# VisualComputingInstitute/diffusion-e2e-ft

Measured on AMD Instinct MI355X. Metric: images/sec (768x768, 1-step UNet fwd) full path: VAE encode + SD-v2 UNet @t=999 + VAE decode, higher is better.
Workload: dtype f16

## Files before the change

### diffusion-e2e-ft_amd/_lib.py

```python
import ctypes as C
import os

import torch

from . import build as _build

_LIB = None

F32, F16, BF16 = 0, 1, 2
_DT = {torch.float32: F32, torch.float16: F16, torch.bfloat16: BF16}


def dtype_id(dt):
    try:
        return _DT[dt]
    except KeyError:
        raise TypeError("libe2eft supports float32/float16/bfloat16, got %s" % dt)


class ConvDesc(C.Structure):
    _fields_ = [(n, C.c_int32) for n in (
        "dtype", "batch", "hin", "win", "hl", "wl", "c1", "ldx1", "c2", "ldx2", "kh", "kw", "stride", "pad_t", "pad_l",
        "hout", "wout", "cout", "ldo", "ldr", "ldw")] + [("alpha", C.c_float)]

# ... 29 lines not shown
class HypersimDesc(C.Structure):
    _fields_ = [(n, C.c_int32) for n in ("batch", "height", "width", "color_dtype", "distance_dtype", "depth_format")] + [
        ("focal", C.c_double), ("scale_numerator", C.c_double)]


HYPERSIM_DEPTH_U16, HYPERSIM_DEPTH_F32 = range(2)
HYPERSIM_RECORD = 16


class DepthGtDesc(C.Structure):
    _fields_ = ([(n, C.c_int32) for n in ("batch", "h0", "w0", "raw_dtype")] + [("divisor", C.c_double)]
                + [(n, C.c_int32) for n in ("inf_to_zero", "crop_top", "crop_left", "crop_h", "crop_w")] + [("min_depth", C.c_float), ("max_depth", C.c_float)]
                + [(n, C.c_int32) for n in ("win_y0", "win_y1", "win_x0", "win_x1", "use_ext_mask")])


GT_U16, GT_I32, GT_F32 = range(3)


class NormalGtDesc(C.Structure):
    _fields_ = [(n, C.c_int32) for n in ("batch", "height", "width", "raw_dtype")]


NORMAL_GT_U8, NORMAL_GT_F32 = range(2)


class DsineRgbDesc(C.Structure):
    _fields_ = [(n, C.c_int32) for n in ("batch", "height", "width", "out_layout")]


RGB_HWC, RGB_CHW = range(2)
DSINE_RGB_WS_INTS = 6


OPT_PERSISTENT, OPT_PERSISTENT_GRID, OPT_NARROW_CONV, OPT_NARROW_MFMA, OPT_IGEMM_GENERAL_OPERANDS, OPT_IGEMM2_WAVES, OPT_PATCH_CONV, OPT_THIN_INPUT_CONV, OPT_FUSED_NORM, OPT_ATTN_DMA, OPT_UPCONV_PHASES, OPT_PATCH_CONV_2X2, OPT_PERSISTENT_MIN_QROUNDS, OPT_GN_APPLY_ITERS, OPT_F32_SPLIT, OPT_F32_SPLIT_ATTN = range(16)

_P = C.c_void_p
_I = C.c_int32
_L = C.c_int64
_F = C.c_float
_Z = C.c_size_t

SIGNATURES = {
    "e2eft_version": (_I, []),
    "e2eft_last_error": (C.c_char_p, []),
    "e2eft_build_id": (C.c_char_p, []),
    "e2eft_set_option": (_I, [_I, _I]),
    "e2eft_get_option": (_I, [_I]),
    "e2eft_conv2d_fwd": (_I, [C.POINTER(ConvDesc), _P, _P, _P, _P, _P, _P, _P, _P]),
    "e2eft_gemm": (_I, [C.POINTER(GemmDesc), _P, _P, _P, _P, _P, _P]),
    "e2eft_conv2d_fwd_gnstats": (_I, [C.POINTER(ConvDesc), _P, _P, _P, _P, _P, _P, _P, _P, _Z, C.POINTER(C.c_int32), _P]),
    "e2eft_conv2d_splitk_workspace_bytes": (_Z, [C.POINTER(ConvDesc)]),
    "e2eft_conv2d_fwd_splitk": (_I, [C.POINTER(ConvDesc), _P, _P, _P, _P, _P, _P, _P, _P, _Z, _P]),
    "e2eft_gemm_gnstats": (_I, [C.POINTER(GemmDesc), _P, _P, _P, _P, _P, _I, _P, _Z, C.POINTER(C.c_int32), _P]),
    "e2eft_groupnorm_fwd_pre": (_I, [C.POINTER(GroupNormDesc), _P, _P, _P, _P, _P, _P, _I, _P, _I, _P, _Z, _P]),
    "e2eft_groupnorm_coeff_offset": (_Z, [C.POINTER(GroupNormDesc)]),
    "e2eft_groupnorm_fwd_stats": (_I, [C.POINTER(GroupNormDesc), _P, _P, _P, _P, _I, _P, _I, _P, _Z, _P]),
    "e2eft_conv2d_fwd_normed_supported": (_I, [C.POINTER(ConvDesc)]),
    "e2eft_upconv2x_fwd_supported": (_I, [C.POINTER(ConvDesc)]),
    "e2eft_upconv2x_fwd": (_I, [C.POINTER(ConvDesc), _P, _P, _P, _P, _P, _Z, C.POINTER(C.c_int32), _P]),
    "e2eft_groupnorm_fwd_split": (_I, [C.POINTER(GroupNormDesc), _P, _P, _P, _P, _I, _P, _P, _I, _P, _Z, _P]),
    "e2eft_f32_split_weight": (_I, [_P, _L, _I, _P, _P, _P]),
    "e2eft_f32_split2_cat": (_I, [_P, _I, _I, _P, _I, _I, _L, _P, _I, _P, _P]),
    "e2eft_f32_split2": (_I, [_P, _L, _I, _I, _P, _I, _P, _P]),
    "e2eft_f32_split2_cols": (_I, [_P, _I, _I, _P, _I, _I, _L, _P, _I, _P, _P]),
    "e2eft_f32_split_wgrad_finish": (_I, [_P, _P, _P, _L, _I, _I, _P, _P, _P, _P]),
    "e2eft_conv2d_fwd_f32split_supported": (_I, [C.POINTER(ConvDesc)]),
    "e2eft_conv2d_fwd_f32split": (_I, [C.POINTER(ConvDesc), _P, _P, _P, _P, _P, _P, _P, _P, _Z, C.POINTER(C.c_int32), _P]),
    "e2eft_upconv2x_fwd_f32split_supported": (_I, [C.POINTER(ConvDesc)]),
    "e2eft_upconv2x_fwd_f32split": (_I, [C.POINTER(ConvDesc), _P, _P, _P, _P, _P, _P, _P, _Z, C.POINTER(C.c_int32), _P]),
    "e2eft_gemm_f32split_supported": (_I, [C.POINTER(GemmDesc)]),
    "e2eft_attn_f32split_supported": (_I, [C.POINTER(AttnDesc), _I]),
    "e2eft_gemm_f32split": (_I, [C.POINTER(GemmDesc), _P, _P, _P, _P, _P, _P, _P, _P]),
    "e2eft_conv2d_fwd_normed": (_I, [C.POINTER(ConvDesc), _P, _P, _P, _I, _P, _P, _P, _P, _P, _P, _Z, C.POINTER(C.c_int32), _P]),
    "e2eft_groupnorm_workspace_bytes": (_Z, [C.POINTER(GroupNormDesc)]),
    "e2eft_groupnorm_fwd": (_I, [C.POINTER(GroupNormDesc), _P, _P, _P, _P, _P, _P, _Z, _P]),
    "e2eft_layernorm_fwd": (_I, [_I, _L, _I, _I, _I, _F, _P, _P, _P, _P, _P]),
    "e2eft_geglu_fwd": (_I, [_I, _L, _I, _I, _I, _P, _P, _P]),
    "e2eft_softmax_rows": (_I, [_I, _L, _I, _L, _F, _P, _P]),
    "e2eft_softmax_rows_causal": (_I, [_I, _L, _I, _L, _F, _I, _P, _P]),
    "e2eft_attn_fwd": (_I, [C.POINTER(AttnDesc), _P, _P, _P, _P, _P]),
    "e2eft_attn_fwd_lse": (_I, [C.POINTER(AttnDesc), _P, _P, _P, _P, _P, _P]),
    "e2eft_attn512_workspace_bytes": (_Z, [C.POINTER(AttnDesc)]),
    "e2eft_attn512_fwd": (_I, [C.POINTER(AttnDesc), _P, _P, _P, _P, _P, _Z, _P]),
    "e2eft_attn_bwd_workspace_bytes": (_Z, [C.POINTER(AttnDesc)]),
    "e2eft_attn_bwd": (_I, [C.POINTER(AttnDesc), _P, _P, _P, _P, _P, _I, _P, _P, _I, _P, _I, _P, _I, _P, _Z, _P]),
    "e2eft_nchw_to_nhwc": (_I, [_I, _I, _I, _I, _I, _I, _I, _F, _F, _P, _P, _P]),
    "e2eft_nhwc_to_nchw": (_I, [_I, _I, _I, _I, _I, _I, _F, _F, _P, _P, _P]),
    "e2eft_copy_scale": (_I, [_I, _L, _I, _I, _I, _F, _F, _P, _P, _P]),
    "e2eft_add": (_I, [_I, _L, _I, _I, _I, _I, _P, _P, _P, _P]),
    "e2eft_timestep_embedding": (_I, [_I, _I, _I, _P, _P, _P]),
    "e2eft_silu": (_I, [_I, _L, _P, _P, _P]),
    "e2eft_depth_head": (_I, [_I, _I, _L, _I, _I, _P, _P, _P]),
    "e2eft_normal_head": (_I, [_I, _I, _I, _I, _I, _I, _F, _P, _P, _P]),
    "e2eft_ssi_loss_workspace_bytes": (_Z, [_I]),
    "e2eft_ssi_loss_fwd": (_I, [_I, _I, _P, _P, _P, _P, _P, _P, _Z, _P]),
    "e2eft_angular_loss_workspace_bytes": (_Z, [_I]),
    "e2eft_angular_loss_fwd": (_I, [_I, _I, _P, _P, _P, _P, _P, _Z, _P]),
    "e2eft_conv2d_dgrad": (_I, [C.POINTER(ConvDesc), _P, _I, _I, _P, _I, _P, _I, _P]),
    "e2eft_conv2d_wgrad_workspace_bytes": (_Z, [C.POINTER(ConvDesc), _I]),
    "e2eft_conv2d_wgrad": (_I, [C.POINTER(ConvDesc), _P, _I, _P, _P, _P, _Z, C.POINTER(C.c_int32), _P]),
    "e2eft_conv2d_im2col_t": (_I, [C.POINTER(ConvDesc), _P, _P, _P, _L, _P]),
    "e2eft_transpose": (_I, [_I, _I, _L, _I, _L, _L, _L, _L, _L, _P, _P, _P]),
    "e2eft_colsum_workspace_bytes": (_Z, [_I, _L, _I]),
    "e2eft_colsum": (_I, [_I, _I, _L, _I, _L, _F, _P, _P, _P, _Z, _P]),
    "e2eft_upsample_nearest_bwd": (_I, [_I, _I, _I, _I, _I, _I, _I, _I, _I, _P, _P, _P]),
    "e2eft_groupnorm_bwd_workspace_bytes": (_Z, [C.POINTER(GroupNormDesc)]),
    "e2eft_groupnorm_bwd": (_I, [C.POINTER(GroupNormDesc), _P, _P, _P, _P, _P, _I, _P, _I, _P, _P, _P, _P, _Z, _P]),
    "e2eft_groupnorm_bwd_add": (_I, [C.POINTER(GroupNormDesc), _P, _P, _P, _P, _P, _I, _P, _I, _P, _I, _P, _P, _P, _P, _Z, _P]),
    "e2eft_layernorm_bwd_workspace_bytes": (_Z, [_L, _I]),
# ... 117 lines not shown
```

### diffusion-e2e-ft_amd/build.py

```python
import hashlib
import os
import shutil
import subprocess
import sys
from concurrent.futures import ThreadPoolExecutor

HERE = os.path.dirname(os.path.abspath(__file__))
CSRC = os.path.join(HERE, "csrc")
LIBDIR = os.path.join(HERE, "lib")
OBJDIR = os.path.join(HERE, "build")
LIB = os.path.join(LIBDIR, "libe2eft.so")
SOURCES = ["api.hip", "igemm.hip", "igemm2.hip", "igemm5.hip", "igemm6.hip", "convin.hip", "norm.hip", "attn.hip", "attn32.hip", "attn512.hip", "attn_bwd.hip", "elementwise.hip", "loss.hip", "bwd.hip", "wgrad.hip", "ensemble.hip", "dataprep.hip", "narrow.hip", "dataaug.hip", "evalmetrics.hip", "normaleval.hip", "d2nt.hip", "hypersimprep.hip", "evalprep.hip", "normalprep.hip", "prepost.hip", "f32split.hip", "attn_f32split.hip", "noise.hip"]
FLAGS = ["--offload-arch=gfx950", "-O3", "-std=c++17", "-fPIC", "-fvisibility=hidden", "-Wall", "-Wno-unused-function"]
EXTRA_FLAGS = {"attn.hip": ["-fno-slp-vectorize"], "attn32.hip": ["-fno-slp-vectorize"], "attn_f32split.hip": ["-fno-slp-vectorize"], "attn512.hip": ["-fno-slp-vectorize"], "igemm.hip": ["-fno-slp-vectorize"], "igemm2.hip": ["-fno-slp-vectorize"], "igemm5.hip": ["-fno-slp-vectorize"], "igemm6.hip": ["-fno-slp-vectorize"], "f32split.hip": ["-fno-slp-vectorize"], "convin.hip": ["-fno-slp-vectorize"],
               "d2nt.hip": ["-ffp-contract=off"],
               "hypersimprep.hip": ["-ffp-contract=off"],
               "evalprep.hip": ["-ffp-contract=off"],
               "normalprep.hip": ["-ffp-contract=off"]}


def _hipcc():
    for cand in (os.environ.get("HIPCC"), shutil.which("hipcc"), "/opt/rocm/bin/hipcc"):
        if cand and os.path.exists(cand):
            return cand
    raise RuntimeError("hipcc not found (need ROCm >= 7.0 to build libe2eft.so for gfx950)")


HEADERS = ["common.h", "gfx950.h", "igemm.h", "attn32.h", "attn512_regs.inc", "igemm_persistent_epilogue.inc"]


def _inputs():
    inc = os.path.join(HERE, "..", "include")
    return [os.path.join(CSRC, f) for f in sorted(SOURCES + HEADERS)] + [os.path.join(inc, "e2eft.h"), os.path.join(inc, "e2eft_debug.h")]


def _newest_source_mtime():
    return max(os.path.getmtime(p) for p in _inputs() + [os.path.abspath(__file__)])


ID_MARK = b"E2EFT_BUILD_ID="


def source_id():
    h = hashlib.sha256()
    for path in _inputs():
# ... 102 lines not shown
```

### diffusion-e2e-ft_amd/csrc/api.hip

```cpp
#include "common.h"
#include <atomic>

namespace e2eft {

static thread_local char g_err[512] = "";

char* err_buf() { return g_err; }

int fail(int code, const char* fmt, ...) {
    va_list ap;
    va_start(ap, fmt);
    vsnprintf(g_err, sizeof(g_err), fmt, ap);
    va_end(ap);
    return code;
}

int check_launch(const char* what) {
    hipError_t e = hipGetLastError();
    if (e != hipSuccess) return fail(E2EFT_ERR_LAUNCH, "%s: launch failed: %s", what, hipGetErrorString(e));
    return E2EFT_OK;
}

static std::atomic<int> g_cus_of_device[64];
int device_cus() {
    int dev = 0;
    if (hipGetDevice(&dev) != hipSuccess || dev < 0 || dev >= 64) return 0;
    int n = g_cus_of_device[dev].load(std::memory_order_relaxed);
    if (n == 0) {
        if (hipDeviceGetAttribute(&n, hipDeviceAttributeMultiprocessorCount, dev) != hipSuccess || n < 8) return 0;
        n &= ~7;
        g_cus_of_device[dev].store(n, std::memory_order_relaxed);
    }
    return n;
}

static thread_local char g_tag[96] = "";
void tag_kernel(const char* fmt, ...) {
    va_list ap;
    va_start(ap, fmt);
    vsnprintf(g_tag, sizeof(g_tag), fmt, ap);
    va_end(ap);
}
const char* last_tag() { return g_tag; }

static std::atomic<int> g_opt[E2EFT_OPT_COUNT] = {{1}, {0}, {1}, {1}, {0}, {0}, {1}, {1}, {1}, {1}, {1}, {1}, {2}, {0}, {1}, {0}};

int option(int key) { return g_opt[key].load(std::memory_order_relaxed); }

}

extern "C" int e2eft_set_option(int32_t key, int32_t value) {
    using namespace e2eft;
    E2EFT_REQUIRE(key >= 0 && key < E2EFT_OPT_COUNT, "set_option: unknown key %d", key);
    bool ok = value == 0 || value == 1;
    if (key == E2EFT_OPT_PERSISTENT_GRID) ok = value == 0 || (value >= 8 && value % 8 == 0 && value <= 4096);
    if (key == E2EFT_OPT_IGEMM2_WAVES) ok = value == 0 || value == 4 || value == 8;
    if (key == E2EFT_OPT_PERSISTENT_MIN_QROUNDS) ok = value >= 1 && value <= 64;
    if (key == E2EFT_OPT_GN_APPLY_ITERS) ok = value >= 0 && value <= 16;
    E2EFT_REQUIRE(ok, "set_option: value %d out of range for key %d", value, key);
    g_opt[key].store(value, std::memory_order_relaxed);
    return E2EFT_OK;
}
extern "C" int e2eft_get_option(int32_t key) { return key >= 0 && key < E2EFT_OPT_COUNT ? e2eft::option(key) : -1; }

extern "C" const char* e2eft_debug_last_kernel(void) { return e2eft::last_tag(); }

extern "C" int e2eft_version(void) { return E2EFT_VERSION; }
#ifndef E2EFT_BUILD_ID
#define E2EFT_BUILD_ID "unstamped"
#endif
static const char k_build_id[] = "E2EFT_BUILD_ID=" E2EFT_BUILD_ID;
extern "C" const char* e2eft_build_id(void) { return k_build_id + 15; }
extern "C" const char* e2eft_last_error(void) { return e2eft::err_buf(); }
```

### diffusion-e2e-ft_amd/modules.py

```python

import torch
from torch import nn

from . import ops
from . import autograd as F


_cached = F.cached


def packed_conv_weight(conv):
    return F.packed_conv_weight(conv, conv.weight.dtype)


def conv_nhwc(conv, x, x2=None, up_to=None, rowadd=None, residual=None, alpha=1.0, pad=None, out=None, gn_stats=True, norm=None):
    assert out is None
    return F.conv(conv, x, x2=x2, up_to=up_to, rowadd=rowadd, residual=residual, alpha=alpha, pad=pad, gn_stats=gn_stats, norm=norm)


def checkpointed(enabled, fn, *args):
    if enabled and torch.is_grad_enabled() and any(isinstance(a, torch.Tensor) and a.requires_grad for a in args):
        from torch.utils.checkpoint import checkpoint
        return checkpoint(fn, *args, use_reentrant=False)
    return fn(*args)
# ... 167 lines not shown
    ops.softmax_rows_(s.view(-1, nkp), nkt, scale)
    o = torch.empty((B, N, C), dtype=dt, device=dev)
    for qh in range(nseg):
        ops.bgemm_raw(dt, N, d, nkp, s[qh * Bv:], nkp, (heads * N * nkp, N * nkp), vt, nkp, (C * nkp, d * nkp), o[qh * Bv:], C, (N * C, d),
                      Bv, heads)
    return o


class Attention(nn.Module):

    def __init__(self, query_dim, heads, cross_attention_dim=None, bias=False, joint=False):
        super().__init__()
        self.heads = heads
        self.scale = (query_dim // heads) ** -0.5
        self.joint = joint
        kv = cross_attention_dim or query_dim
        self.to_q = Linear(query_dim, query_dim, bias=bias)
        self.to_k = Linear(kv, query_dim, bias=bias)
        self.to_v = Linear(kv, query_dim, bias=bias)
        self.to_out = nn.ModuleList([Linear(query_dim, query_dim), nn.Dropout(0.0)])

    def forward(self, x, ctx=None, residual=None):
        B, N, C = x.shape
        d = C // self.heads
        out = self.to_out[0]
        kv_pre = None
        shared_src = None
        if isinstance(ctx, CtxCond):
            kv_pre = ctx.kv.get(id(self))
            shared_src = ctx.src if ctx.shared else None
            ctx = ctx.ctx
        if F.needs_grad(x, ctx, self.to_q.weight, self.to_k.weight, self.to_v.weight, out.weight):
            return out(self._forward_train(x, ctx), residual=residual)
        if (CROSS_ATTN_FOLD and shared_src is not None and shared_src.shape[1] == 2 and not self.joint and self.to_q.bias is None and self.to_k.bias is None
                and self.to_v.bias is None and self.heads <= 64):
            return self._folded(x, shared_src, residual)
        fused = F.fused_attention_ok(x.dtype, d)
        dt = x.dtype
        if fused:
            if ctx is None:
                qkv = F.linear(x, (self.to_q.weight, self.to_k.weight, self.to_v.weight), owner=self, name="wqkv")
                q, k, v = qkv[..., :C], qkv[..., C:2 * C], qkv[..., 2 * C:]
            else:
                q = self.to_q(x)
                kv = kv_pre
                if kv is None or torch.is_grad_enabled():
                    kv = F.linear(ctx, (self.to_k.weight, self.to_v.weight), owner=self, name="wkv")
                k, v = kv[..., :C], kv[..., C:]
            a = ops.attention(q, k, v, self.heads, self.scale, kv_nseg=2 if self.joint else 1, kv_bmod=B // 2 if self.joint else B)
        else:
            src = x if ctx is None else ctx
            cw = lambda lin: F._cat_weight(lin, "w", (lin.weight,), dt, lin.weight.shape[1])
            a = attention_unfused(x, src, cw(self.to_q), F._vec(self.to_q.bias, dt), cw(self.to_k), F._vec(self.to_k.bias, dt), cw(self.to_v),
                                  F._vec(self.to_v.bias, dt), self.heads, self.scale, joint=self.joint)
        return out(a, residual=residual)

    def _fold(self, src, dt):
        out = self.to_out[0]
        ws = [w for w in (self.to_q.weight, self.to_k.weight, self.to_v.weight, out.weight, out.bias) if w is not None]
        key = (src.data_ptr(), src._version, tuple(src.shape), str(src.device), dt, F._key(*ws))
        hit = self.__dict__.get("_fold_cache")
        if hit is not None and hit[0] == key:
            return hit[1]
        with torch.no_grad():
            h, C = self.heads, self.to_q.weight.shape[0]
            d = C // h
            f32 = lambda w: w.detach().float().contiguous()
            wq, wk, wv, wo = f32(self.to_q.weight), f32(self.to_k.weight), f32(self.to_v.weight), f32(out.weight)
            c32 = f32(src[0])
            k = ops.gemm(c32, wk)
            v = ops.gemm(c32, wv)
            ar = torch.arange(h, device=k.device)
            Mk = torch.zeros((h, h, d), dtype=torch.float32, device=k.device)
            Mv = torch.zeros((h, h, d), dtype=torch.float32, device=k.device)
            Mk[ar, ar] = (k[0] - k[1]).view(h, d) * self.scale
            Mv[ar, ar] = (v[0] - v[1]).view(h, d)
            G = ops.gemm(Mk.view(h, C), wq.t().contiguous())
            delta = ops.gemm(Mv.view(h, C), wo)
            c0 = ops.gemm(v[1:2].contiguous(), wo, f32(out.bias) if out.bias is not None else None)[0]
            hp = ops.round_up(h, ops.epc(dt))
            Gp = torch.zeros((hp, C), dtype=torch.float32, device=G.device)
            Gp[:h] = G
            Dt = torch.zeros((C, hp), dtype=torch.float32, device=G.device)
            Dt[:, :h] = delta.t()
            val = (Gp.to(dt).contiguous(), Dt.to(dt).contiguous(), c0.to(dt).contiguous())
        self.__dict__["_fold_cache"] = (key, val, src)
        return val

    def _folded(self, x, src, residual):
        G, Dt, c0 = self._fold(src, x.dtype)
        p = ops.activation(ops.linear(x, G), "sigmoid")
        return ops.linear(p, Dt, c0, residual=residual)

    def _forward_train(self, x, ctx):
        B, N, C = x.shape
        if ctx is None:
            bias = None if self.to_q.bias is None else torch.cat([self.to_q.bias, self.to_k.bias, self.to_v.bias])
            qkv = F.linear(x, (self.to_q.weight, self.to_k.weight, self.to_v.weight), bias, owner=self, name="wqkv")
            if self.joint:
                Bv = B // 2
                q, kv = qkv[..., :C], qkv[..., C:]
                kv = torch.cat([kv[:Bv], kv[Bv:]], dim=1).repeat(2, 1, 1)
                return F.attention(q.contiguous(), kv, self.heads, self.scale)
            return F.attention(qkv, None, self.heads, self.scale)
        q = self.to_q(x)
        bias = None if self.to_k.bias is None else torch.cat([self.to_k.bias, self.to_v.bias])
        kv = F.linear(ctx, (self.to_k.weight, self.to_v.weight), bias, owner=self, name="wkv")
        return F.attention(q, kv, self.heads, self.scale)


class GEGLU(nn.Module):

    def __init__(self, dim, inner):
        super().__init__()
        self.proj = Linear(dim, 2 * inner)

    def forward(self, x):
        return F.geglu(self.proj(x))


class FeedForward(nn.Module):

    def __init__(self, dim):
        super().__init__()
        self.net = nn.ModuleList([GEGLU(dim, 4 * dim), nn.Dropout(0.0), Linear(4 * dim, dim)])

    def forward(self, x, residual=None):
        return self.net[2](self.net[0](x), residual=residual)


class BasicTransformerBlock(nn.Module):

    def __init__(self, dim, heads, cross_attention_dim, joint=False):
        super().__init__()
        self.norm1 = LayerNorm(dim, eps=1e-5)
        self.attn1 = Attention(dim, heads, joint=joint)
        self.norm2 = LayerNorm(dim, eps=1e-5)
        self.attn2 = Attention(dim, heads, cross_attention_dim=cross_attention_dim)
        self.norm3 = LayerNorm(dim, eps=1e-5)
        self.ff = FeedForward(dim)

    def forward(self, h, ctx):
        h = self.attn1(self.norm1(h), None, residual=h)
        h = self.attn2(self.norm2(h), ctx, residual=h)
        return self.ff(self.norm3(h), residual=h)


class Transformer2DModel(nn.Module):

    def __init__(self, channels, heads, cross_attention_dim, groups=32, joint=False):
        super().__init__()
        self.norm = GroupNorm(groups, channels, eps=1e-6, affine=True)
        self.proj_in = Linear(channels, channels)
        self.transformer_blocks = nn.ModuleList([BasicTransformerBlock(channels, heads, cross_attention_dim, joint=joint)])
        self.proj_out = Linear(channels, channels)

    def nhwc(self, x, ctx):
        B, H, W, C = x.shape
        h, x = self.norm.nhwc(x, split=True)
        h = self.proj_in(h.view(B, H * W, C))
        for blk in self.transformer_blocks:
            h = blk(h, ctx)
        out = self.proj_out(h, residual=x.reshape(B, H * W, C), gn_rows_per_image=H * W)
        res = out.view(B, H, W, C)
        st = getattr(out, "_e2eft_gn", None)
        if st is not None:
            res._e2eft_gn = st
        return res


class VaeAttention(nn.Module):

    def __init__(self, channels, groups=32):
        super().__init__()
        self.group_norm = GroupNorm(groups, channels, eps=1e-6, affine=True)
        self.to_q = Linear(channels, channels)
        self.to_k = Linear(channels, channels)
        self.to_v = Linear(channels, channels)
# ... 28 lines not shown
```

### diffusion-e2e-ft_amd/ops.py

```python
import ctypes as C

import torch

from . import _lib
from ._lib import ConvDesc, GemmDesc, GroupNormDesc, AttnDesc, check, dtype_id


class KernelTimer:

    def __init__(self, only=None):
        self.rec = {}
        self.only = only

    def add(self, name, start, end, flops, nbytes, label=None, launches=1, flops_nominal=None):
        self.rec.setdefault(name, []).append((start, end, flops, nbytes, label, launches, flops if flops_nominal is None else flops_nominal))

    def summary(self):
        torch.cuda.synchronize()
        out = {}
        for name, lst in self.rec.items():
            ms = sum(r[0].elapsed_time(r[1]) for r in lst)
            out[name] = dict(launches=sum(r[5] for r in lst), ms=ms, flops=float(sum(r[2] for r in lst)), bytes=float(sum(r[3] for r in lst)),
                             flops_nominal=float(sum(r[6] for r in lst)))
        return out
# ... 579 lines not shown


NORM_FUSION_ENABLED = True


def groupnorm_stats(x, gamma, groups, eps):
    _check_cuda(x, gamma)
    B, H, W, c1 = x.shape
    d = GroupNormDesc()
    d.dtype = dtype_id(x.dtype)
    d.batch, d.hw = B, H * W
    d.c1, d.ldx1, d.c2, d.ldx2 = c1, _nhwc_ld(x), 0, 0
    d.groups, d.ldy, d.silu, d.eps = groups, c1, 0, eps
    lib = _lib.load()
    nbytes = lib.e2eft_groupnorm_workspace_bytes(C.byref(d))
    if nbytes == 0:
        raise RuntimeError("groupnorm_stats: %s" % lib.e2eft_last_error().decode())
    ws = torch.empty((nbytes + 3) // 4, dtype=torch.float32, device=x.device)
    s1 = getattr(x, "_e2eft_gn", None) if GN_STATS_ENABLED else None
    with _timed("groupnorm_stats", 0.0, 0.0, label="gn stats B%d %dx%d C%d" % (B, H, W, c1)):
        check(lib.e2eft_groupnorm_fwd_stats(C.byref(d), _ptr(x), C.c_void_p(0), _ptr(gamma), _ptr(s1.partial) if s1 else C.c_void_p(0), s1.nslabs if s1 else 0,
                                            C.c_void_p(0), 0, _ptr(ws), nbytes, _stream()))
    return ws, ws.data_ptr() + lib.e2eft_groupnorm_coeff_offset(C.byref(d))


def layernorm(x, gamma, beta, eps, out=None):
    _check_cuda(x, gamma, beta, out)
    Cc = x.shape[-1]
    a = x.reshape(-1, Cc) if x.is_contiguous() else _as_rows(x)
    if out is None:
        out = torch.empty(x.shape, dtype=x.dtype, device=x.device)
    o = out.reshape(-1, Cc) if out.is_contiguous() else _as_rows(out)
    assert gamma.dtype == x.dtype and beta.dtype == x.dtype
    check(_lib.load().e2eft_layernorm_fwd(dtype_id(x.dtype), a.shape[0], Cc, _rows_ld(a), _rows_ld(o), eps, _ptr(a), _ptr(gamma),
                                         _ptr(beta), _ptr(o), _stream()))
    return out


def geglu(h, out=None):
    _check_cuda(h, out)
    c2 = h.shape[-1]
    c = c2 // 2
    a = h.reshape(-1, c2) if h.is_contiguous() else _as_rows(h)
    if out is None:
        out = torch.empty((*h.shape[:-1], c), dtype=h.dtype, device=h.device)
    o = out.reshape(-1, c) if out.is_contiguous() else _as_rows(out)
    check(_lib.load().e2eft_geglu_fwd(dtype_id(h.dtype), a.shape[0], c, _rows_ld(a), _rows_ld(o), _ptr(a), _ptr(o), _stream()))
    return out


def softmax_rows_(s, n, scale, causal_nq=0):
    _check_cuda(s)
    assert s.dim() == 2 and s.is_contiguous()
    if causal_nq:
        check(_lib.load().e2eft_softmax_rows_causal(dtype_id(s.dtype), s.shape[0], n, s.shape[1], scale, causal_nq, _ptr(s), _stream()))
    else:
        check(_lib.load().e2eft_softmax_rows(dtype_id(s.dtype), s.shape[0], n, s.shape[1], scale, _ptr(s), _stream()))
    return s


def _ld3(t):
    if t.shape[2] > 1 and t.stride(2) != 1:
        raise ValueError("attention operands need unit inner stride")
    ld = t.stride(1) if t.shape[1] > 1 else max(t.shape[2], t.stride(1))
    if t.shape[0] > 1 and t.stride(0) != t.shape[1] * ld:
        raise ValueError("attention operands must be batch-dense: %s %s" % (tuple(t.shape), t.stride()))
    return ld


def _attn_desc(q, k, v, out, heads, scale, kv_nseg, kv_bmod):
    B, Nq, Wd = q.shape
    Bkv, Nk, _ = k.shape
    assert Wd == heads * 64 and k.shape[2] == Wd and v.shape == k.shape
    d = AttnDesc()
    d.dtype = dtype_id(q.dtype)
    d.batch, d.heads, d.nq, d.nk_seg = B, heads, Nq, Nk
    d.kv_nseg = kv_nseg
    d.kv_bmod = B if kv_bmod is None else kv_bmod
    assert Bkv >= d.kv_bmod * kv_nseg
    d.ldq, d.ldk, d.ldv, d.ldo = _ld3(q), _ld3(k), _ld3(v), _ld3(out)
# ... 118 lines not shown
    _check_cuda(a, b, out)
    assert a.shape == b.shape and a.dtype == b.dtype
    if out is None:
        out = torch.empty(a.shape, dtype=a.dtype, device=a.device)
    Cc = a.shape[-1]
    aa, bb, oo = (_as_rows(t) if t.dim() > 2 else t for t in (a, b, out))
    check(_lib.load().e2eft_add(dtype_id(a.dtype), aa.shape[0], Cc, _rows_ld(aa), _rows_ld(bb), _rows_ld(oo), _ptr(aa), _ptr(bb), _ptr(oo), _stream()))
    return out


def timestep_embedding(t, dim, dtype):
    _check_cuda(t)
    t = t.to(torch.int64).contiguous()
    out = torch.empty((t.shape[0], dim), dtype=dtype, device=t.device)
    check(_lib.load().e2eft_timestep_embedding(dtype_id(dtype), t.shape[0], dim, _ptr(t), _ptr(out), _stream()))
    return out


def silu(x):
    _check_cuda(x)
    x = x.contiguous()
    out = torch.empty_like(x)
    check(_lib.load().e2eft_silu(dtype_id(x.dtype), x.numel(), _ptr(x), _ptr(out), _stream()))
    return out


ACT_KINDS = {"quick_gelu": 0, "gelu": 1, "silu": 2, "sigmoid": 3}


def activation(x, kind):
    _check_cuda(x)
    x = x.contiguous()
    out = torch.empty_like(x)
    check(_lib.load().e2eft_activation(dtype_id(x.dtype), ACT_KINDS[kind], x.numel(), _ptr(x), _ptr(out), _stream()))
    return out


def depth_head(x, to_unit, dtype=None):
    _check_cuda(x)
    B, H, W, _ = x.shape
    dtype = dtype or x.dtype
    y = torch.empty((B, 1, H, W), dtype=dtype, device=x.device)
    mode = 2 if to_unit == "mean" else (1 if to_unit else 0)
    check(_lib.load().e2eft_depth_head(dtype_id(x.dtype), dtype_id(dtype), B * H * W, _nhwc_ld(x), mode, _ptr(x), _ptr(y), _stream()))
    return y


def normal_head(x, clamp=False, sign=1.0, dtype=None):
    _check_cuda(x)
    B, H, W, _ = x.shape
    dtype = dtype or x.dtype
    y = torch.empty((B, 3, H, W), dtype=dtype, device=x.device)
    check(_lib.load().e2eft_normal_head(dtype_id(x.dtype), dtype_id(dtype), B, H * W, _nhwc_ld(x), 1 if clamp else 0, sign, _ptr(x), _ptr(y), _stream()))
    return y


def ssi_loss(pred, target, mask, return_scale_shift=False):
    _check_cuda(pred, target, mask)
    B = pred.shape[0]
    p = pred.reshape(B, -1).float().contiguous()
    t = target.reshape(B, -1).float().contiguous()
    m = mask.reshape(B, -1).to(torch.uint8).contiguous()
    lib = _lib.load()
    nbytes = lib.e2eft_ssi_loss_workspace_bytes(B)
    ws = torch.empty((nbytes + 7) // 8, dtype=torch.float64, device=p.device)
    out = torch.empty(1, dtype=torch.float32, device=p.device)
    ss = torch.empty((B, 2), dtype=torch.float32, device=p.device)
# ... 831 lines not shown
```

### include/e2eft.h

```cpp
#ifndef E2EFT_H
#define E2EFT_H

#include <stddef.h>
#include <stdint.h>

#ifdef __cplusplus
extern "C" {
#endif
#pragma GCC visibility push(default)

#define E2EFT_VERSION 119

enum {
    E2EFT_OK = 0,
    E2EFT_ERR_BAD_ARG = 1,
    E2EFT_ERR_WORKSPACE = 2,
    E2EFT_ERR_LAUNCH = 3,
    E2EFT_ERR_UNSUPPORTED = 4,
};

enum { E2EFT_F32 = 0, E2EFT_F16 = 1, E2EFT_BF16 = 2 };

int e2eft_version(void);
const char* e2eft_last_error(void);
const char* e2eft_build_id(void);

enum {
    E2EFT_OPT_PERSISTENT = 0,
    E2EFT_OPT_PERSISTENT_GRID = 1,
    E2EFT_OPT_NARROW_CONV = 2,
    E2EFT_OPT_NARROW_MFMA = 3,
    E2EFT_OPT_IGEMM_GENERAL_OPERANDS = 4,
    E2EFT_OPT_IGEMM2_WAVES = 5,
    E2EFT_OPT_PATCH_CONV = 6,
    E2EFT_OPT_THIN_INPUT_CONV = 7,
    E2EFT_OPT_FUSED_NORM = 8,
    E2EFT_OPT_ATTN_DMA = 9,
    E2EFT_OPT_UPCONV_PHASES = 10,
    E2EFT_OPT_PATCH_CONV_2X2 = 11,
    E2EFT_OPT_PERSISTENT_MIN_QROUNDS = 12,
    E2EFT_OPT_GN_APPLY_ITERS = 13,
    E2EFT_OPT_F32_SPLIT = 14,
    E2EFT_OPT_F32_SPLIT_ATTN = 15,
    E2EFT_OPT_COUNT = 16
};
int e2eft_set_option(int32_t key, int32_t value);
int e2eft_get_option(int32_t key);

typedef struct E2eftConvDesc {
    int32_t dtype;
    int32_t batch, hin, win, hl, wl;
    int32_t c1, ldx1;
    int32_t c2, ldx2;
    int32_t kh, kw, stride;
    int32_t pad_t, pad_l;
    int32_t hout, wout;
    int32_t cout, ldo;
    int32_t ldr;
    int32_t ldw;
    float alpha;
} E2eftConvDesc;

int e2eft_conv2d_fwd(const E2eftConvDesc* d, const void* x1, const void* x2, const void* w,
                     const void* bias ,
                     const void* rowadd ,
                     const void* residual , void* out, void* stream);

typedef struct E2eftGemmDesc {
    int32_t dtype;
    int32_t m, n, k;
    int32_t lda, ldw, ldo, ldr;
    int32_t nzo, nzi;
    int64_t sa_o, sa_i, sw_o, sw_i, so_o, so_i, sr_o, sr_i;
    int32_t bias_along_m;
    float alpha;
} E2eftGemmDesc;

// ... 31 lines not shown
size_t e2eft_conv2d_splitk_workspace_bytes(const E2eftConvDesc* d);
int e2eft_conv2d_fwd_splitk(const E2eftConvDesc* d, const void* x1, const void* x2, const void* w, const void* bias,
                            const void* rowadd, const void* residual, void* out, void* workspace, size_t ws_bytes, void* stream);
int e2eft_gemm_gnstats(const E2eftGemmDesc* d, const void* a, const void* w, const void* bias, const void* residual,
                       void* out, int32_t rows_per_image, float* gn_partial, size_t gn_partial_bytes,
                       int32_t* slab_rows, void* stream);

typedef struct E2eftGroupNormDesc {
    int32_t dtype;
    int32_t batch, hw;
    int32_t c1, ldx1, c2, ldx2;
    int32_t groups;
    int32_t ldy;
    int32_t silu;
    float eps;
} E2eftGroupNormDesc;

size_t e2eft_groupnorm_workspace_bytes(const E2eftGroupNormDesc* d);
int e2eft_groupnorm_fwd(const E2eftGroupNormDesc* d, const void* x1, const void* x2, const void* gamma,
                        const void* beta, void* y, void* workspace, size_t ws_bytes, void* stream);

int e2eft_groupnorm_fwd_split(const E2eftGroupNormDesc* d, const float* x, const float* gamma, const float* beta, void* planes, int32_t ldp, float* scale,
                              const float* partial1, int32_t nslabs1, void* workspace, size_t ws_bytes, void* stream);

int e2eft_groupnorm_fwd_pre(const E2eftGroupNormDesc* d, const void* x1, const void* x2, const void* gamma,
                            const void* beta, void* y, const float* partial1, int32_t nslabs1, const float* partial2,
                            int32_t nslabs2, void* workspace, size_t ws_bytes, void* stream);
size_t e2eft_groupnorm_coeff_offset(const E2eftGroupNormDesc* d);
int e2eft_groupnorm_fwd_stats(const E2eftGroupNormDesc* d, const void* x1, const void* x2, const void* gamma, const float* partial1,
                              int32_t nslabs1, const float* partial2, int32_t nslabs2, void* workspace, size_t ws_bytes, void* stream);

int e2eft_layernorm_fwd(int32_t dtype, int64_t rows, int32_t c, int32_t ldx, int32_t ldy, float eps,
                        const void* x, const void* gamma, const void* beta, void* y, void* stream);

int e2eft_geglu_fwd(int32_t dtype, int64_t rows, int32_t c, int32_t ldh, int32_t ldy, const void* h, void* y,
                    void* stream);

int e2eft_softmax_rows(int32_t dtype, int64_t rows, int32_t n, int64_t lds, float scale, void* s, void* stream);
int e2eft_softmax_rows_causal(int32_t dtype, int64_t rows, int32_t n, int64_t lds, float scale, int32_t nq, void* s, void* stream);

typedef struct E2eftAttnDesc {
    int32_t dtype;
    int32_t batch, heads, nq, nk_seg;
    int32_t kv_nseg, kv_bmod;
    int32_t ldq, ldk, ldv, ldo;
    float scale;
} E2eftAttnDesc;

int e2eft_attn_fwd(const E2eftAttnDesc* d, const void* q, const void* k, const void* v, void* out, void* stream);
int e2eft_attn_fwd_lse(const E2eftAttnDesc* d, const void* q, const void* k, const void* v, void* out, float* lse, void* stream);
int32_t e2eft_attn_f32split_supported(const E2eftAttnDesc* d, int32_t backward);
size_t e2eft_attn512_workspace_bytes(const E2eftAttnDesc* d);
int e2eft_attn512_fwd(const E2eftAttnDesc* d, const void* q, const void* k, const void* v, void* out, void* workspace, size_t ws_bytes,
                      void* stream);
size_t e2eft_conv2d_wgrad_workspace_bytes(const E2eftConvDesc* d, int32_t lddy);
int e2eft_conv2d_wgrad(const E2eftConvDesc* d, const void* dy, int32_t lddy, const void* x1, const void* x2, float* partial, size_t partial_bytes,
                       int32_t* nsplit_out, void* stream);
size_t e2eft_attn_bwd_workspace_bytes(const E2eftAttnDesc* d);
int e2eft_attn_bwd(const E2eftAttnDesc* d, const void* q, const void* k, const void* v, const void* out, const void* dout,
                   int32_t lddo, const float* lse, void* dq, int32_t lddq, void* dk, int32_t lddk, void* dv, int32_t lddv,
                   void* workspace, size_t ws_bytes, void* stream);


int e2eft_nchw_to_nhwc(int32_t dt_in, int32_t dt_out, int32_t batch, int32_t c, int32_t hw, int32_t cpad,
                       int32_t ldy, float mul, float add, const void* x, void* y, void* stream);
int e2eft_nhwc_to_nchw(int32_t dt_in, int32_t dt_out, int32_t batch, int32_t c, int32_t hw, int32_t ldx,
// ... 172 lines not shown
```

Measured before the change: 89.53.

## Fuse norm2, folded cross-attention, residual and norm3 into one row kernel

Adds a row-wise HIP kernel that runs the second LayerNorm, the folded two-token cross-attention (sigmoid gate over a small head projection G, then mixing of delta rows plus c0), the residual add and the third LayerNorm in a single pass, holding G and delta in LDS. The transformer block uses it when the context is shared and folding applies, replacing separate layernorm, linear, activation, linear and layernorm launches and their intermediate global-memory round trips. It also adds timing wrappers to several elementwise ops. The risk is that per-row CUDA-core dot products against up to 32 head rows run slower than the MFMA GEMMs they replace, and LDS use limits occupancy.

```diff
diff --git a/diffusion-e2e-ft_amd/_lib.py b/diffusion-e2e-ft_amd/_lib.py
--- a/diffusion-e2e-ft_amd/_lib.py
+++ b/diffusion-e2e-ft_amd/_lib.py
@@ -85,7 +85,7 @@
 DSINE_RGB_WS_INTS = 6
 
 
-OPT_PERSISTENT, OPT_PERSISTENT_GRID, OPT_NARROW_CONV, OPT_NARROW_MFMA, OPT_IGEMM_GENERAL_OPERANDS, OPT_IGEMM2_WAVES, OPT_PATCH_CONV, OPT_THIN_INPUT_CONV, OPT_FUSED_NORM, OPT_ATTN_DMA, OPT_UPCONV_PHASES, OPT_PATCH_CONV_2X2, OPT_PERSISTENT_MIN_QROUNDS, OPT_GN_APPLY_ITERS, OPT_F32_SPLIT, OPT_F32_SPLIT_ATTN = range(16)
+OPT_PERSISTENT, OPT_PERSISTENT_GRID, OPT_NARROW_CONV, OPT_NARROW_MFMA, OPT_IGEMM_GENERAL_OPERANDS, OPT_IGEMM2_WAVES, OPT_PATCH_CONV, OPT_THIN_INPUT_CONV, OPT_FUSED_NORM, OPT_ATTN_DMA, OPT_UPCONV_PHASES, OPT_PATCH_CONV_2X2, OPT_PERSISTENT_MIN_QROUNDS, OPT_GN_APPLY_ITERS, OPT_F32_SPLIT, OPT_F32_SPLIT_ATTN, OPT_XATTN_ROWS = range(17)
 
 _P = C.c_void_p
 _I = C.c_int32
@@ -128,6 +128,8 @@
     "e2eft_groupnorm_workspace_bytes": (_Z, [C.POINTER(GroupNormDesc)]),
     "e2eft_groupnorm_fwd": (_I, [C.POINTER(GroupNormDesc), _P, _P, _P, _P, _P, _P, _Z, _P]),
     "e2eft_layernorm_fwd": (_I, [_I, _L, _I, _I, _I, _F, _P, _P, _P, _P, _P]),
+    "e2eft_xattn2_rows_supported": (_I, [_I, _L, _I, _I, _I, _I, _I]),
+    "e2eft_xattn2_rows_fwd": (_I, [_I, _L, _I, _I, _P, _I, _P, _P, _F, _P, _P, _P, _P, _P, _F, _P, _I, _P, _I, _P]),
     "e2eft_geglu_fwd": (_I, [_I, _L, _I, _I, _I, _P, _P, _P]),
     "e2eft_softmax_rows": (_I, [_I, _L, _I, _L, _F, _P, _P]),
     "e2eft_softmax_rows_causal": (_I, [_I, _L, _I, _L, _F, _I, _P, _P]),
diff --git a/diffusion-e2e-ft_amd/build.py b/diffusion-e2e-ft_amd/build.py
--- a/diffusion-e2e-ft_amd/build.py
+++ b/diffusion-e2e-ft_amd/build.py
@@ -10,7 +10,7 @@
 LIBDIR = os.path.join(HERE, "lib")
 OBJDIR = os.path.join(HERE, "build")
 LIB = os.path.join(LIBDIR, "libe2eft.so")
-SOURCES = ["api.hip", "igemm.hip", "igemm2.hip", "igemm5.hip", "igemm6.hip", "convin.hip", "norm.hip", "attn.hip", "attn32.hip", "attn512.hip", "attn_bwd.hip", "elementwise.hip", "loss.hip", "bwd.hip", "wgrad.hip", "ensemble.hip", "dataprep.hip", "narrow.hip", "dataaug.hip", "evalmetrics.hip", "normaleval.hip", "d2nt.hip", "hypersimprep.hip", "evalprep.hip", "normalprep.hip", "prepost.hip", "f32split.hip", "attn_f32split.hip", "noise.hip"]
+SOURCES = ["api.hip", "igemm.hip", "igemm2.hip", "igemm5.hip", "igemm6.hip", "convin.hip", "norm.hip", "attn.hip", "attn32.hip", "attn512.hip", "attn_bwd.hip", "elementwise.hip", "loss.hip", "bwd.hip", "wgrad.hip", "ensemble.hip", "dataprep.hip", "narrow.hip", "dataaug.hip", "evalmetrics.hip", "normaleval.hip", "d2nt.hip", "hypersimprep.hip", "evalprep.hip", "normalprep.hip", "prepost.hip", "f32split.hip", "attn_f32split.hip", "noise.hip", "xattn_rows.hip"]
 FLAGS = ["--offload-arch=gfx950", "-O3", "-std=c++17", "-fPIC", "-fvisibility=hidden", "-Wall", "-Wno-unused-function"]
 EXTRA_FLAGS = {"attn.hip": ["-fno-slp-vectorize"], "attn32.hip": ["-fno-slp-vectorize"], "attn_f32split.hip": ["-fno-slp-vectorize"], "attn512.hip": ["-fno-slp-vectorize"], "igemm.hip": ["-fno-slp-vectorize"], "igemm2.hip": ["-fno-slp-vectorize"], "igemm5.hip": ["-fno-slp-vectorize"], "igemm6.hip": ["-fno-slp-vectorize"], "f32split.hip": ["-fno-slp-vectorize"], "convin.hip": ["-fno-slp-vectorize"],
                "d2nt.hip": ["-ffp-contract=off"],
diff --git a/diffusion-e2e-ft_amd/csrc/api.hip b/diffusion-e2e-ft_amd/csrc/api.hip
--- a/diffusion-e2e-ft_amd/csrc/api.hip
+++ b/diffusion-e2e-ft_amd/csrc/api.hip
@@ -43,7 +43,7 @@
 }
 const char* last_tag() { return g_tag; }
 
-static std::atomic<int> g_opt[E2EFT_OPT_COUNT] = {{1}, {0}, {1}, {1}, {0}, {0}, {1}, {1}, {1}, {1}, {1}, {1}, {2}, {0}, {1}, {0}};
+static std::atomic<int> g_opt[E2EFT_OPT_COUNT] = {{1}, {0}, {1}, {1}, {0}, {0}, {1}, {1}, {1}, {1}, {1}, {1}, {2}, {0}, {1}, {0}, {1}};
 
 int option(int key) { return g_opt[key].load(std::memory_order_relaxed); }
 
diff --git a/diffusion-e2e-ft_amd/csrc/xattn_rows.hip b/diffusion-e2e-ft_amd/csrc/xattn_rows.hip
--- /dev/null
+++ b/diffusion-e2e-ft_amd/csrc/xattn_rows.hip
@@ -0,0 +1,266 @@
+#include "common.h"
+
+namespace e2eft {
+
+struct XrArgs {
+    long rows;
+    int rpw;
+    int C, hp, ldh, ldo, ldn;
+    float eps2, eps3;
+    const void *h, *gamma2, *beta2, *G, *delta, *c0, *gamma3, *beta3;
+    void *out, *n3;
+};
+
+template <int L>
+__device__ __forceinline__ float row_sum(float v) {
+#pragma unroll
+    for (int o = L / 2; o > 0; o >>= 1) v += __shfl_xor(v, o, 64);
+    return v;
+}
+
+template <typename T>
+__device__ __forceinline__ void xr_stage(T* dst, const int stride, const T* __restrict__ src, const int nrows, const int nchunks, const int tid, const int nt) {
+    for (int k = tid; k < nrows * nchunks; k += nt) {
+        const int r = k / nchunks, c = k - r * nchunks;
+        *reinterpret_cast<u32x4*>(dst + r * stride + c * 8) = *reinterpret_cast<const u32x4*>(src + k * 8);
+    }
+}
+
+constexpr int XR_MAXI = 5;
+#define XR_FENCE() asm volatile("" ::: "memory")
+
+constexpr int xr_lds_bytes(int L, int HPG) { return (2 * 8 * HPG + 5) * (L * XR_MAXI * 8) * 2; }
+
+template <typename T, int L, int NT, int HPG>
+__global__ __launch_bounds__(NT) __attribute__((amdgpu_waves_per_eu(HPG == 4 ? 2 : 4, HPG == 4 ? 2 : 4))) void xattn2_rows_kernel(const XrArgs a) {
+    constexpr int EPC = 8, MAXI = XR_MAXI, RPP = NT / L, HP = 8 * HPG, CS = L * XR_MAXI * 8, FJ = HPG >= 3 ? 2 : 4;
+    static_assert((2 * HP + 5) * CS * 2 == xr_lds_bytes(L, HPG) && HP * CS * 2 + 5 * L * 16 <= 65536, "LDS image");
+    static_assert(sizeof(T) == 2, "16-bit tensors");
+    static_assert(xr_lds_bytes(L, HPG) <= 163840, "LDS");
+    __shared__ __attribute__((aligned(16))) unsigned char smem[xr_lds_bytes(L, HPG)];
+    const int C = a.C, nchunks = C / EPC;
+    T* const sG = reinterpret_cast<T*>(smem);
+    T* const sD = sG + HP * CS;
+    T* const sV = sD + HP * CS;
+    const int tid = threadIdx.x, l = tid % L, slot = tid / L;
+    const long row0 = (long)blockIdx.x * a.rpw;
+    const long rend = min(row0 + (long)a.rpw, a.rows);
+    const T* __restrict__ h = (const T*)a.h;
+    T* __restrict__ out = (T*)a.out;
+    T* __restrict__ n3 = (T*)a.n3;
+
+    xr_stage(sG, CS, (const T*)a.G, HP, nchunks, tid, NT);
+    xr_stage(sD, CS, (const T*)a.delta, HP, nchunks, tid, NT);
+    xr_stage(sV, CS, (const T*)a.c0, 1, nchunks, tid, NT);
+    xr_stage(sV + CS, CS, (const T*)a.gamma2, 1, nchunks, tid, NT);
+    xr_stage(sV + 2 * CS, CS, (const T*)a.beta2, 1, nchunks, tid, NT);
+    if (n3) {
+        xr_stage(sV + 3 * CS, CS, (const T*)a.gamma3, 1, nchunks, tid, NT);
+        xr_stage(sV + 4 * CS, CS, (const T*)a.beta3, 1, nchunks, tid, NT);
+    }
+    __syncthreads();
+
+    const float invc = 1.f / (float)C;
+    for (long row = row0 + slot; row < rend; row += RPP) {
+        Vec16<T> hr[MAXI], n2[MAXI];
+#pragma unroll
+        for (int i = 0; i < MAXI; ++i) {
+            if (l + L * i < nchunks) hr[i] = ld16(h + row * a.ldh + (l + L * i) * EPC);
+            else hr[i].raw = u32x4{0u, 0u, 0u, 0u};
+        }
+        float sum = 0.f;
+#pragma unroll
+        for (int i = 0; i < MAXI; ++i) {
+            if (l + L * i < nchunks) {
+#pragma unroll
+                for (int e = 0; e < EPC; ++e) sum += to_f(hr[i].e[e]);
+            }
+        }
+        const float mean = row_sum<L>(sum) * invc;
+        float sq = 0.f;
+#pragma unroll
+        for (int i = 0; i < MAXI; ++i) {
+            if (l + L * i < nchunks) {
+#pragma unroll
+                for (int e = 0; e < EPC; ++e) { const float dd = to_f(hr[i].e[e]) - mean; sq += dd * dd; }
+            }
+        }
+        const float rstd = rsqrtf(row_sum<L>(sq) * invc + a.eps2);
+#pragma unroll
+        for (int i = 0; i < MAXI; ++i) {
+            const int ch = l + L * i;
+            if (ch < nchunks) {
+                const Vec16<T> ga = ld16(sV + CS + ch * EPC), be = ld16(sV + 2 * CS + ch * EPC);
+#pragma unroll
+                for (int e = 0; e < EPC; ++e) n2[i].e[e] = from_f<T>((to_f(hr[i].e[e]) - mean) * rstd * to_f(ga.e[e]) + to_f(be.e[e]));
+            } else {
+                n2[i].raw = u32x4{0u, 0u, 0u, 0u};
+            }
+        }
+        float p[HP];
+#pragma unroll
+        for (int g = 0; g < HP; g += 8) {
+            float lg[8];
+#pragma unroll
+            for (int j = 0; j < 8; ++j) lg[j] = 0.f;
+#pragma unroll
+            for (int i = 0; i < MAXI; ++i) {
+                const int ch = l + L * i;
+                if (ch < nchunks) {
+                    asm volatile("" : "+v"(n2[i].raw));
+                    float nf[EPC];
+#pragma unroll
+                    for (int e = 0; e < EPC; ++e) nf[e] = to_f(n2[i].e[e]);
+#pragma unroll
+                    for (int j = 0; j < 8; ++j) {
+                        const Vec16<T> gv = ld16(sG + (g + j) * CS + ch * EPC);
+#pragma unroll
+                        for (int e = 0; e < EPC; ++e) lg[j] = fmaf(nf[e], to_f(gv.e[e]), lg[j]);
+                        if (j % FJ == FJ - 1) XR_FENCE();
+                    }
+                }
+            }
+#pragma unroll
+            for (int j = 0; j < 8; ++j) {
+                const float s = to_f(from_f<T>(row_sum<L>(lg[j])));
+                p[g + j] = to_f(from_f<T>(__builtin_amdgcn_rcpf(1.0f + __expf(-s))));
+            }
+        }
+        float v[MAXI][EPC];
+#pragma unroll
+        for (int i = 0; i < MAXI; ++i) {
+            const int ch = l + L * i;
+            if (ch < nchunks) {
+                asm volatile("" : "+v"(hr[i].raw));
+                const Vec16<T> cc = ld16(sV + ch * EPC);
+#pragma unroll
+                for (int e = 0; e < EPC; ++e) v[i][e] = to_f(hr[i].e[e]) + to_f(cc.e[e]);
+            } else {
+#pragma unroll
+                for (int e = 0; e < EPC; ++e) v[i][e] = 0.f;
+            }
+        }
+#pragma unroll
+        for (int g = 0; g < HP; g += 8) {
+#pragma unroll
+            for (int i = 0; i < MAXI; ++i) {
+                const int ch = l + L * i;
+                if (ch < nchunks) {
+#pragma unroll
+                    for (int j = 0; j < 8; ++j) {
+                        const Vec16<T> dv = ld16(sD + (g + j) * CS + ch * EPC);
+#pragma unroll
+                        for (int e = 0; e < EPC; ++e) v[i][e] = fmaf(p[g + j], to_f(dv.e[e]), v[i][e]);
+                        if (j % FJ == FJ - 1) XR_FENCE();
+                    }
+                }
+            }
+        }
+        sum = 0.f;
+#pragma unroll
+        for (int i = 0; i < MAXI; ++i) {
+            const int ch = l + L * i;
+            if (ch < nchunks) {
+                Vec16<T> o;
+#pragma unroll
+                for (int e = 0; e < EPC; ++e) {
+                    o.e[e] = from_f<T>(v[i][e]);
+                    v[i][e] = to_f(o.e[e]);
+                    sum += v[i][e];
+                }
+                st16(out + row * a.ldo + ch * EPC, o);
+            }
+        }
+        if (n3) {
+            const float mean3 = row_sum<L>(sum) * invc;
+            sq = 0.f;
+#pragma unroll
+            for (int i = 0; i < MAXI; ++i) {
+                if (l + L * i < nchunks) {
+#pragma unroll
+                    for (int e = 0; e < EPC; ++e) { const float dd = v[i][e] - mean3; sq += dd * dd; }
+                }
+            }
+            const float rstd3 = rsqrtf(row_sum<L>(sq) * invc + a.eps3);
+#pragma unroll
+            for (int i = 0; i < MAXI; ++i) {
+                const int ch = l + L * i;
+                if (ch < nchunks) {
+                    const Vec16<T> ga = ld16(sV + 3 * CS + ch * EPC), be = ld16(sV + 4 * CS + ch * EPC);
+                    Vec16<T> o;
+#pragma unroll
+                    for (int e = 0; e < EPC; ++e) o.e[e] = from_f<T>((v[i][e] - mean3) * rstd3 * to_f(ga.e[e]) + to_f(be.e[e]));
+                    st16(n3 + row * a.ldn + ch * EPC, o);
+                }
+            }
+        }
+    }
+}
+
+struct XrPlan {
+    int L, nt, wpc;
+};
+static bool xr_plan(int C, int hp, XrPlan& p) {
+    const int nchunks = C / 8;
+    if (nchunks <= 8 * XR_MAXI) p = {8, 256, 4};
+    else if (nchunks <= 16 * XR_MAXI) p = {16, 512, 2};
+    else if (nchunks <= 32 * XR_MAXI) p = {32, 1024, 1};
+    else if (nchunks <= 64 * XR_MAXI) p = {64, 1024, 1};
+    else return false;
+    return xr_lds_bytes(p.L, hp / 8) <= 163840;
+}
+
+}
+
+using namespace e2eft;
+
+extern "C" int32_t e2eft_xattn2_rows_supported(int32_t dtype, int64_t rows, int32_t C, int32_t hp, int32_t ldh, int32_t ldo, int32_t ldn) {
+    if (!option(E2EFT_OPT_XATTN_ROWS)) return 0;
+    if (dtype != E2EFT_F16 && dtype != E2EFT_BF16) return 0;
+    if (rows < 1 || rows >= 2147483647L || C < 8 || C % 8 != 0 || hp < 8 || hp > 32 || hp % 8 != 0) return 0;
+    if (ldh < C || ldh % 8 != 0 || ldo < C || ldo % 8 != 0 || (ldn != 0 && (ldn < C || ldn % 8 != 0))) return 0;
+    XrPlan p;
+    return xr_plan(C, hp, p) ? 1 : 0;
+}
+
+extern "C" int e2eft_xattn2_rows_fwd(int32_t dtype, int64_t rows, int32_t C, int32_t hp, const void* h, int32_t ldh, const void* gamma2, const void* beta2, float eps2,
+                                     const void* G, const void* delta, const void* c0, const void* gamma3, const void* beta3, float eps3, void* out, int32_t ldo,
+                                     void* n3, int32_t ldn, void* stream) {
+    E2EFT_REQUIRE(h && gamma2 && beta2 && G && delta && c0 && out, "xattn2_rows: null pointer");
+    E2EFT_REQUIRE(n3 ? (gamma3 && beta3 && ldn != 0) : ldn == 0, "xattn2_rows: n3 needs gamma3, beta3 and ldn; without n3, ldn is 0");
+    if (!e2eft_xattn2_rows_supported(dtype, rows, C, hp, ldh, ldo, ldn))
+        return fail(E2EFT_ERR_UNSUPPORTED, "xattn2_rows: dtype=%d rows=%ld C=%d hp=%d ldh=%d ldo=%d ldn=%d is not served (ask e2eft_xattn2_rows_supported)", (int)dtype, (long)rows,
+                    (int)C, (int)hp, (int)ldh, (int)ldo, (int)ldn);
+    E2EFT_REQUIRE(al16(h) && al16(gamma2) && al16(beta2) && al16(G) && al16(delta) && al16(c0) && al16(out) && al16(n3) && al16(gamma3) && al16(beta3),
+                  "xattn2_rows: pointers must be 16-byte aligned");
+    XrPlan p;
+    xr_plan(C, hp, p);
+    int cus = device_cus();
+    if (cus <= 0) cus = 256;
+    const long rpp = p.nt / p.L, target = (long)cus * p.wpc;
+    const long passes = (rows + target * rpp - 1) / (target * rpp);
+    long rpw = passes > 1 ? passes * rpp : (rows + target - 1) / target;
+    if (rpw < 8) rpw = 8;
+    const long nwg = (rows + rpw - 1) / rpw;
+    XrArgs a;
+    a.rows = rows; a.rpw = (int)rpw;
+    a.C = C; a.hp = hp; a.ldh = ldh; a.ldo = ldo; a.ldn = ldn;
+    a.eps2 = eps2; a.eps3 = eps3;
+    a.h = h; a.gamma2 = gamma2; a.beta2 = beta2; a.G = G; a.delta = delta; a.c0 = c0; a.gamma3 = gamma3; a.beta3 = beta3;
+    a.out = out; a.n3 = n3;
+    hipStream_t s = (hipStream_t)stream;
+    const int hpg = hp / 8;
+#define XR_LAUNCH(T, LL, NT, HPG) hipLaunchKernelGGL((xattn2_rows_kernel<T, LL, NT, HPG>), dim3((unsigned)nwg), dim3(NT), 0, s, a)
+#define XR_DISPATCH(T)                                                                                                       \
+    do {                                                                                                                     \
+        if (p.L == 8) { if (hpg == 1) XR_LAUNCH(T, 8, 256, 1); else if (hpg == 2) XR_LAUNCH(T, 8, 256, 2); else if (hpg == 3) XR_LAUNCH(T, 8, 256, 3); else XR_LAUNCH(T, 8, 256, 4); } \
+        else if (p.L == 16) { if (hpg == 1) XR_LAUNCH(T, 16, 512, 1); else if (hpg == 2) XR_LAUNCH(T, 16, 512, 2); else if (hpg == 3) XR_LAUNCH(T, 16, 512, 3); else XR_LAUNCH(T, 16, 512, 4); } \
+        else if (p.L == 32) { if (hpg == 1) XR_LAUNCH(T, 32, 1024, 1); else if (hpg == 2) XR_LAUNCH(T, 32, 1024, 2); else XR_LAUNCH(T, 32, 1024, 3); } \
+        else XR_LAUNCH(T, 64, 1024, 1);                                                                                      \
+    } while (0)
+    if (dtype == E2EFT_F16) XR_DISPATCH(f16);
+    else XR_DISPATCH(bf16);
+#undef XR_DISPATCH
+#undef XR_LAUNCH
+    return check_launch("xattn2_rows");
+}
diff --git a/diffusion-e2e-ft_amd/modules.py b/diffusion-e2e-ft_amd/modules.py
--- a/diffusion-e2e-ft_amd/modules.py
+++ b/diffusion-e2e-ft_amd/modules.py
@@ -223,8 +223,7 @@
             ctx = ctx.ctx
         if F.needs_grad(x, ctx, self.to_q.weight, self.to_k.weight, self.to_v.weight, out.weight):
             return out(self._forward_train(x, ctx), residual=residual)
-        if (CROSS_ATTN_FOLD and shared_src is not None and shared_src.shape[1] == 2 and not self.joint and self.to_q.bias is None and self.to_k.bias is None
-                and self.to_v.bias is None and self.heads <= 64):
+        if self._fold_ok(shared_src):
             return self._folded(x, shared_src, residual)
         fused = F.fused_attention_ok(x.dtype, d)
         dt = x.dtype
@@ -278,6 +277,18 @@
         self.__dict__["_fold_cache"] = (key, val, src)
         return val
 
+    def _fold_ok(self, shared_src):
+        return (CROSS_ATTN_FOLD and shared_src is not None and shared_src.shape[1] == 2 and not self.joint and self.to_q.bias is None and self.to_k.bias is None
+                and self.to_v.bias is None and self.heads <= 64)
+
+    def _fold_rows(self, src, dt):
+        G, Dt, c0 = self._fold(src, dt)
+        entry = self.__dict__["_fold_cache"]
+        if len(entry) < 4:
+            entry = entry + (Dt.t().contiguous(),)
+            self.__dict__["_fold_cache"] = entry
+        return G, entry[3], c0
+
     def _folded(self, x, src, residual):
         G, Dt, c0 = self._fold(src, x.dtype)
         p = ops.activation(ops.linear(x, G), "sigmoid")
@@ -333,8 +344,31 @@
 
     def forward(self, h, ctx):
         h = self.attn1(self.norm1(h), None, residual=h)
+        rows = self._xattn_rows(h, ctx)
+        if rows is not None:
+            return self.ff(rows[1], residual=rows[0])
         h = self.attn2(self.norm2(h), ctx, residual=h)
         return self.ff(self.norm3(h), residual=h)
+
+    def _xattn_rows(self, h, ctx):
+        att = self.attn2
+        if not isinstance(ctx, CtxCond) or not ctx.shared or not att._fold_ok(ctx.src) or h.dtype == torch.float32:
+            return None
+        out = att.to_out[0]
+        if F.needs_grad(h, ctx.ctx, att.to_q.weight, att.to_k.weight, att.to_v.weight, out.weight, out.bias, self.norm2.weight, self.norm2.bias, self.norm3.weight,
+                        self.norm3.bias):
+            return None
+        C = h.shape[-1]
+        if not h.is_contiguous() or h.dim() < 2:
+            return None
+        rows = h.numel() // C
+        hp = ops.round_up(att.heads, ops.epc(h.dtype))
+        if not ops.xattn2_rows_supported(h.dtype, rows, C, hp, C, C, C):
+            return None
+        G, delta, c0 = att._fold_rows(ctx.src, h.dtype)
+        dt = h.dtype
+        return ops.xattn2_rows(h, F._vec(self.norm2.weight, dt), F._vec(self.norm2.bias, dt), self.norm2.eps, G, delta, c0,
+                               F._vec(self.norm3.weight, dt), F._vec(self.norm3.bias, dt), self.norm3.eps)
 
 
 class Transformer2DModel(nn.Module):
diff --git a/diffusion-e2e-ft_amd/ops.py b/diffusion-e2e-ft_amd/ops.py
--- a/diffusion-e2e-ft_amd/ops.py
+++ b/diffusion-e2e-ft_amd/ops.py
@@ -635,9 +635,39 @@
         out = torch.empty(x.shape, dtype=x.dtype, device=x.device)
     o = out.reshape(-1, Cc) if out.is_contiguous() else _as_rows(out)
     assert gamma.dtype == x.dtype and beta.dtype == x.dtype
-    check(_lib.load().e2eft_layernorm_fwd(dtype_id(x.dtype), a.shape[0], Cc, _rows_ld(a), _rows_ld(o), eps, _ptr(a), _ptr(gamma),
-                                         _ptr(beta), _ptr(o), _stream()))
-    return out
+    with _timed("layernorm", 0.0, 2.0 * a.shape[0] * Cc * x.element_size(), label="layernorm M%d C%d" % (a.shape[0], Cc)):
+        check(_lib.load().e2eft_layernorm_fwd(dtype_id(x.dtype), a.shape[0], Cc, _rows_ld(a), _rows_ld(o), eps, _ptr(a), _ptr(gamma),
+                                             _ptr(beta), _ptr(o), _stream()))
+    return out
+
+
+def xattn2_rows_supported(dtype, rows, Cc, hp, ldh, ldo, ldn):
+    return _lib.load().e2eft_xattn2_rows_supported(dtype_id(dtype), rows, Cc, hp, ldh, ldo, ldn) == 1
+
+
+def xattn2_rows(h, gamma2, beta2, eps2, G, delta, c0, gamma3=None, beta3=None, eps3=0.0, out=None, n3=None):
+    _check_cuda(h, gamma2, beta2, G, delta, c0, gamma3, beta3, out, n3)
+    Cc = h.shape[-1]
+    hp = G.shape[0]
+    a = h.reshape(-1, Cc) if h.is_contiguous() else _as_rows(h)
+    want_n3 = gamma3 is not None
+    assert tuple(G.shape) == (hp, Cc) and tuple(delta.shape) == (hp, Cc) and G.is_contiguous() and delta.is_contiguous() and c0.numel() == Cc
+    assert all(t is None or (t.dtype == h.dtype and t.is_contiguous()) for t in (gamma2, beta2, G, delta, c0, gamma3, beta3)) and (beta3 is not None) == want_n3
+    if out is None:
+        out = torch.empty(h.shape, dtype=h.dtype, device=h.device)
+    o = out.reshape(-1, Cc) if out.is_contiguous() else _as_rows(out)
+    n = None
+    if want_n3:
+        if n3 is None:
+            n3 = torch.empty(h.shape, dtype=h.dtype, device=h.device)
+        n = n3.reshape(-1, Cc) if n3.is_contiguous() else _as_rows(n3)
+    else:
+        n3 = None
+    rows = a.shape[0]
+    with _timed("xattn_rows", 4.0 * rows * Cc * hp, (3.0 if want_n3 else 2.0) * rows * Cc * h.element_size(), label="xattn_rows M%d C%d H%d" % (rows, Cc, hp)):
+        check(_lib.load().e2eft_xattn2_rows_fwd(dtype_id(h.dtype), rows, Cc, hp, _ptr(a), _rows_ld(a), _ptr(gamma2), _ptr(beta2), eps2, _ptr(G), _ptr(delta), _ptr(c0),
+                                               _ptr(gamma3), _ptr(beta3), eps3, _ptr(o), _rows_ld(o), _ptr(n), _rows_ld(n) if want_n3 else 0, _stream()))
+    return out, n3
 
 
 def geglu(h, out=None):
@@ -648,7 +678,8 @@
     if out is None:
         out = torch.empty((*h.shape[:-1], c), dtype=h.dtype, device=h.device)
     o = out.reshape(-1, c) if out.is_contiguous() else _as_rows(out)
-    check(_lib.load().e2eft_geglu_fwd(dtype_id(h.dtype), a.shape[0], c, _rows_ld(a), _rows_ld(o), _ptr(a), _ptr(o), _stream()))
+    with _timed("geglu", 0.0, 3.0 * a.shape[0] * c * h.element_size(), label="geglu M%d C%d" % (a.shape[0], c)):
+        check(_lib.load().e2eft_geglu_fwd(dtype_id(h.dtype), a.shape[0], c, _rows_ld(a), _rows_ld(o), _ptr(a), _ptr(o), _stream()))
     return out
 
 
@@ -833,7 +864,8 @@
     _check_cuda(x)
     x = x.contiguous()
     out = torch.empty_like(x)
-    check(_lib.load().e2eft_activation(dtype_id(x.dtype), ACT_KINDS[kind], x.numel(), _ptr(x), _ptr(out), _stream()))
+    with _timed("activation", 0.0, 2.0 * x.numel() * x.element_size(), label="%s n%d" % (kind, x.numel())):
+        check(_lib.load().e2eft_activation(dtype_id(x.dtype), ACT_KINDS[kind], x.numel(), _ptr(x), _ptr(out), _stream()))
     return out
 
 
diff --git a/include/e2eft.h b/include/e2eft.h
--- a/include/e2eft.h
+++ b/include/e2eft.h
@@ -42,7 +42,8 @@
     E2EFT_OPT_GN_APPLY_ITERS = 13,
     E2EFT_OPT_F32_SPLIT = 14,
     E2EFT_OPT_F32_SPLIT_ATTN = 15,
-    E2EFT_OPT_COUNT = 16
+    E2EFT_OPT_XATTN_ROWS = 16,
+    E2EFT_OPT_COUNT = 17
 };
 int e2eft_set_option(int32_t key, int32_t value);
 int e2eft_get_option(int32_t key);
@@ -140,6 +141,11 @@
 
 int e2eft_layernorm_fwd(int32_t dtype, int64_t rows, int32_t c, int32_t ldx, int32_t ldy, float eps,
                         const void* x, const void* gamma, const void* beta, void* y, void* stream);
+
+int32_t e2eft_xattn2_rows_supported(int32_t dtype, int64_t rows, int32_t C, int32_t hp, int32_t ldh, int32_t ldo, int32_t ldn);
+int e2eft_xattn2_rows_fwd(int32_t dtype, int64_t rows, int32_t C, int32_t hp, const void* h, int32_t ldh, const void* gamma2, const void* beta2, float eps2,
+                          const void* G, const void* delta, const void* c0, const void* gamma3, const void* beta3, float eps3, void* out, int32_t ldo,
+                          void* n3, int32_t ldn, void* stream);
 
 int e2eft_geglu_fwd(int32_t dtype, int64_t rows, int32_t c, int32_t ldh, int32_t ldy, const void* h, void* y,
                     void* stream);
```

Result: no change. 89.99, median of 6 (+0.5%).
